# lmwdhr/ViT-CNN

Hardware: AMD Instinct MI355X
Metric: training patches/sec, 9×9 HSI(144)+LiDAR patch, batch 64, 1/2/4/8 GPU (higher is better)
Workload: dtype fp32; 1 GPU; ViT-CNN (Multimodality_Mamba) train step, Houston2013 shape 144+1 bands, 9x9, 16 classes; global_batch=64, per_gpu_batch=64, parallelism=dp1, launch=hipGraph (whole step)

## Files before the change

include/vitcnn.h:

```cpp
#ifndef VITCNN_H
#define VITCNN_H

#include <stddef.h>
#include <hip/hip_runtime_api.h>

#ifdef __cplusplus
#define VC_API extern "C" __attribute__((visibility("default")))
#else
#define VC_API __attribute__((visibility("default")))
#endif

VC_API int vc_gemm(int transA, int transB, int M, int N, int K, float alpha,
                   const float* A, long lda, long strideA, const float* B, long ldb, long strideB,
                   float beta, float* C, long ldc, long strideC, int batch,
                   const float* bias, const float* addend, long add_ld, int add_mod, int flags,
                   float* bias_grad, float* ws, long ws_floats, hipStream_t stream);
VC_API int vc_gemm_ex(int transA, int transB, int M, int N, int K, float alpha, const float* A, long lda,
                      long strideA, const float* B, long ldb, long strideB, float beta, float* C, long ldc,
                      long strideC, int batch, const float* bias, const float* addend, long add_ld, int add_mod,
                      int flags, float* bias_grad, float* ws, long ws_floats, unsigned int* tile_counters,
                      int n_counters, hipStream_t stream);

VC_API int vc_gemm_tune(int bm, int bn, int nsplit, int pf, int combine);

// ... 122 lines not shown
                                    float* dA_log, float* dDskip, float* dgate_logits, float* scratch,
                                    long scratch_floats, hipStream_t stream);
VC_API int vc_mamba_dirconv_bwd(int B, int L, int D, int ndir, const int* order, const int* inv_order,
                                const float* xz, const float* conv_w, const float* conv_b, float* du, float* dxz,
                                float* dconv_w, float* dconv_b, float* ws, long ws_floats, hipStream_t stream);
VC_API int vc_mamba_scan_fwd_fused(int B, int L, int D, int R, int ndir, const float* xz, const int* order,
                                   const float* conv_w, const float* conv_b, const float* x_proj_w,
                                   const float* dt_w, const float* dt_b, const float* A_log, const float* Dskip,
                                   float* u, float* xdbl, float* yp, float* ckpt, hipStream_t stream);
VC_API int vc_mamba_scan_bwd_fused(int B, int L, int D, int R, int ndir, const float* u, const float* xdbl,
                                   const int* order, const float* xz, const float* conv_w, const float* conv_b,
                                   const float* x_proj_w, const float* dt_w, const float* dt_b, const float* A_log,
                                   const float* Dskip, const float* gate_logits, const float* yp, const float* dyp,
                                   const float* ckpt, float* dpre, float* ddt_lin, float* dxdbl, float* conv_part,
                                   float* dA_log, float* dDskip, float* dgate_logits, float* ws, long ws_floats,
                                   hipStream_t stream);
VC_API int vc_mamba_dirconv_bwd_gather(int B, int L, int D, int ndir, const int* inv_order, const float* conv_w,
                                       const float* dpre, float* dxz, hipStream_t stream);
VC_API int vc_mamba_conv_params(int B, int D, int ndir, const float* conv_part, float* dconv_w, float* dconv_b,
                                hipStream_t stream);
VC_API int vc_mamba_bwd_params(int B, int D, int ndir, const float* gate_logits, const float* ws, const float* conv_part,
                               float* dA_log, float* dDskip, float* dgate_logits, float* dconv_w, float* dconv_b,
                               hipStream_t stream);

VC_API int vc_rowchain_front(int rows, int K0, int E, int N2, const float* x, const float* w_embed, const float* pos,
                             int L, float* t, const float* ln_w, const float* ln_b, float eps, float* xn, float* mean,
                             float* rstd, const float* w_proj, float* out, hipStream_t stream);
VC_API int vc_rowchain_back(int B, int L, int D, int ndir, const int* inv_order, const float* gate_logits,
                            const float* yp, const float* xz, float* ypsum, float* ysum, int E, const float* w_out,
                            const float* residual, float* t2, const float* ln_w, const float* ln_b, float eps,
                            float* g, float* mean, float* rstd, int N2, const float* w_proj, const float* b_proj,
                            float* out, hipStream_t stream);

VC_API int vc_rowchain_back_bwd(int rows, int Cout, int E, int D, const float* dcd, const float* w_cd, const float* t2,
                                const float* mean, const float* rstd, const float* ln_w, float* dt, float* ln_part,
                                const float* w_out, const float* xz, const float* ypsum, float* dyp, float* dxz,
                                hipStream_t stream);
VC_API int vc_rowchain_front_bwd(int rows, int K0, int E, int Cin, const float* dxz, const float* w_in, const float* t,
                                 const float* mean, const float* rstd, const float* ln_w, const float* res, float* dtt,
                                 float* ln_part, const float* w_embed, float* dx, float beta, const float* dx_add,
                                 hipStream_t stream);
VC_API int vc_rowchain_ln_params(int rows, int E, const float* ln_part, float* dw, float* db, float beta,
                                 hipStream_t stream);
VC_API int vc_rowchain_ln_part_floats(int rows, int E);

VC_API int vc_tl_ws_floats(int B, int HW, int S);
// ... 95 lines not shown
```

vit-cnn_amd/csrc/mamba.hip:

```cpp
#include "common.h"

namespace {

constexpr int NST = 16;

constexpr int DC_T = 8;
__global__ void dirconv_fwd_run(int total, FastDiv fD, FastDiv fC, FastDiv fB, int L, const int* __restrict__ order,
                                const float* __restrict__ xz, const float* __restrict__ cw,
                                const float* __restrict__ cb, float* __restrict__ u) {
  const int idx = blockIdx.x * blockDim.x + threadIdx.x;
  if (idx >= total) return;
  const int D = fD.div;
  int d, c, b;
  const int sc = fdivmod(idx, fD, d);
  const int sq = fdivmod(sc, fC, c);
  const int k = fdivmod(sq, fB, b);
  const int* ord = order + k * L;
  const float* xb = xz + (long)b * L * (2 * D) + d;
  const float w0 = cw[d * 4], w1 = cw[d * 4 + 1], w2 = cw[d * 4 + 2], w3 = cw[d * 4 + 3], bias = cb[d];
  const int t0 = c * DC_T;
  float x[DC_T + 3];
#pragma unroll
  for (int i = 0; i < DC_T + 3; ++i) {
    const int tau = t0 - 3 + i;
// ... 375 lines not shown
  const int l = threadIdx.x & 15;
  const bool b1 = l & 2;
  float z[2];
#if VC_DPP_PAIRWISE
  float y4[4];
#pragma unroll
  for (int j = 0; j < 4; ++j) y4[j] = dpp_pair_add<0>(v[j], v[j + 4]);
#pragma unroll
  for (int j = 0; j < 2; ++j) z[j] = dpp_pair_add<1>(y4[j], y4[j + 2]);
#else
  dpp_stage12(v, z[0], z[1]);
#endif
  const float keep = b1 ? z[1] : z[0], send = b1 ? z[0] : z[1];
  const float w = keep + dpp_mov<0x4E>(send);
  return w + dpp_mov<0xB1>(w);
}

struct FusedBwd {
  const float* xz;
  const float* conv_w;
  const float* conv_b;
  const float* wx;
  float* conv_part;
  int tail;
};

struct ScanBwdOut {
  float* du;
  float* ddtl;
  float* dxdbl;
  float* da_part;
  float* dd_part;
  float* dg_part;
};

template <int RT>
__device__ __forceinline__ void fused_bwd_tail(const ScanArgs& a, const FusedBwd& fb, const ScanBwdOut& o, int s,
                                               int b, const SeqLds& m, const int* ord, float* red, int Lp,
                                               int Dp) {
  const int R = RT ? RT : a.R, XW = R + 2 * NST, D = a.D, L = a.L;
  const int lane = threadIdx.x & 63, wave = threadIdx.x >> 6, nw = blockDim.x >> 6;
  const int r = lane & 15, g = lane >> 4;
  const int ntm = (Lp + 15) / 16, nkc = Dp / 16;
  const long base = (long)s * L;
  float* DX16 = red;
  float* wdt_lds = red + Lp * 16;
  {
    constexpr int WS = 8;
    float wv[WS];
#pragma unroll
    for (int j = 0; j < WS; ++j) {
      const int i = threadIdx.x + j * blockDim.x;
      wv[j] = i < D * R ? a.wdt[i] : 0.f;
    }
#pragma unroll
    for (int j = 0; j < WS; ++j) {
      const int i = threadIdx.x + j * blockDim.x;
      if (i < D * R) wdt_lds[i] = wv[j];
    }
  }
  __syncthreads();
  f32x4 avs[2][FMAX_KC];
  const int nu = (fb.tail & 2) ? 2 : 0;
#pragma unroll
  for (int u = 0; u < 2; ++u) {
    const int ta = 16 * (wave + u * nw) + r;
    const bool tok = ta < L;
// ... 9 lines not shown
  for (int u = 0; u < nu; ++u) {
    const int tm = wave + u * nw;
    if (tm >= ntm) break;
    const f32x4* av = avs[u];
    const bool jok = r < R;
    f32x4 acc = {0.f, 0.f, 0.f, 0.f};
#pragma unroll
    for (int kc = 0; kc < FMAX_KC; ++kc)
      if (kc < nkc) {
        const int k0 = 16 * kc + 4 * g;
        float bv[4];
#pragma unroll
        for (int e = 0; e < 4; ++e) bv[e] = (jok && k0 + e < D) ? wdt_lds[(k0 + e) * R + r] : 0.f;
        acc = __builtin_amdgcn_mfma_f32_16x16x4f32(av[kc].x, bv[0], acc, 0, 0, 0);
        acc = __builtin_amdgcn_mfma_f32_16x16x4f32(av[kc].y, bv[1], acc, 0, 0, 0);
        acc = __builtin_amdgcn_mfma_f32_16x16x4f32(av[kc].z, bv[2], acc, 0, 0, 0);
        acc = __builtin_amdgcn_mfma_f32_16x16x4f32(av[kc].w, bv[3], acc, 0, 0, 0);
      }
#pragma unroll
    for (int i = 0; i < 4; ++i) {
      const int t = 16 * tm + 4 * g + i;
      if (t < Lp) {
        DX16[t * 16 + r] = jok ? acc[i] : 0.f;
        if (jok && t < L) o.dxdbl[(base + t) * XW + r] = acc[i];
      }
    }
  }
  const int dl = 16 * wave + r;
  const bool dok = dl < D;
  const int dcl = dok ? dl : 0;
  f32x4 bw[3];
#pragma unroll
  for (int kc = 0; kc < 3; ++kc)
#pragma unroll
    for (int e = 0; e < 4; ++e) {
      const int jj = 4 * g + e;
      const int j = kc == 0 ? jj : R + 16 * (kc - 1) + jj;
      bw[kc][e] = (dok && (kc > 0 || jj < R)) ? fb.wx[(long)j * D + dcl] : 0.f;
    }
  __syncthreads();
  const unsigned lb = dok ? (unsigned)dl * 4u : 0x80000000u;
  const auto r_dp = buf_rsrc(o.du + base * D, (unsigned)(L * D * 4));
  const float w0 = cf_ld(fb.conv_w, dcl * 4, dok), w1 = cf_ld(fb.conv_w, dcl * 4 + 1, dok),
              w2 = cf_ld(fb.conv_w, dcl * 4 + 2, dok), w3 = cf_ld(fb.conv_w, dcl * 4 + 3, dok),
              bias = cf_ld(fb.conv_b, dcl, dok);
  const float* xb = fb.xz + (long)b * L * (2 * D) + dcl;
  float cacc[5] = {0.f, 0.f, 0.f, 0.f, 0.f};
// ... 40 lines not shown
          pre = fmaf(w2, xv[u][i + 2], pre);
          pre = fmaf(w3, xv[u][i + 3], pre);
          const float sg = sigmoid_f(pre);
          const float du = m.dts[(tq + i) * Dp + dl] + acc[i];
          const float gd = dok ? du * sg * (1.f + pre * (1.f - sg)) : 0.f;
          buf_st(r_dp, (unsigned)((tq + i) * D * 4) + lb, gd);
          cacc[4] += gd;
          cacc[0] += gd * xv[u][i];
          cacc[1] += gd * xv[u][i + 1];
          cacc[2] += gd * xv[u][i + 2];
          cacc[3] += gd * xv[u][i + 3];
        }
      }
    }
  }
#pragma unroll
  for (int e = 0; e < 5; ++e) cacc[e] = cross_row_sum(cacc[e]);
  if (g == 0 && dok) {
    float* cp = fb.conv_part + (long)s * 5 * D;
#pragma unroll
    for (int e = 0; e < 4; ++e) cp[dl * 4 + e] = cacc[e];
    cp[4 * D + dl] = cacc[4];
  }
}

template <int RT, bool BM, bool FUSE>
__global__ __launch_bounds__(512, 4) void scan_bwd(ScanArgs a, int ndir, const float* __restrict__ gate_logits,
                                                const float* __restrict__ yp, const float* __restrict__ dyp,
                                                const float* __restrict__ ckpt, ScanBwdOut o, int rbs,
                                                FusedBwd fb) {
  extern __shared__ __attribute__((aligned(16))) float smem[];
  const int R = RT ? RT : a.R;
  const int XW = R + 2 * NST;
  const int nseg = seg_count(a.L), Lp = nseg * SCK;
  const int nw = blockDim.x >> 6, Dp = nw * 16;
  const SeqLds m(smem, Lp, R, Dp);
  float* red = m.xr + Lp * R;
  const int nbuf = 2 * rbs;
  const int red_n = FUSE ? max(nbuf * nw * SCK * 32, Lp * 16 + a.D * R) : nbuf * nw * SCK * 32;
  int* ord = reinterpret_cast<int*>(red + red_n + nw);
  const int s = blockIdx.x, k = s / a.B, b = s - k * a.B;
  for (int t = threadIdx.x; t < a.L; t += blockDim.x) ord[t] = a.order[k * a.L + t];
  const int lane = threadIdx.x & 63, wave = threadIdx.x >> 6, q = lane >> 4, cl = lane & 15;
  const int d = wave * 16 + cl;
  const bool valid = d < a.D;
  const int dc = valid ? d : 0;
  const float g = gate_softmax(gate_logits, ndir, k);
  float A2[NQ];
#pragma unroll
  for (int j = 0; j < NQ; ++j) A2[j] = valid ? -__expf(a.alog[dc * NST + NQ * q + j]) * LOG2E : 0.f;
  const float Dd = valid ? a.dskip[dc] : 0.f;
  const long base = (long)s * a.L;
  const int vi = cl >> 1;
  const int col = vi < 4 ? NQ * q + vi : NST + NQ * q + vi - 4;
  const f2 A2v[2] = {f2{A2[0], A2[1]}, f2{A2[2], A2[3]}};
  f2 dh[2] = {f2{0.f, 0.f}, f2{0.f, 0.f}}, dAacc[2] = {f2{0.f, 0.f}, f2{0.f, 0.f}};
  float dD_acc = 0.f, dg_acc = 0.f;
  float hn[NQ], un[SCK], dn[SCK], yn[SCK];
  const unsigned seq_bytes = (unsigned)(a.L * a.D * 4);
  const auto r_u = buf_rsrc(a.u + base * a.D, seq_bytes);
  const auto r_yp = buf_rsrc(yp + base * a.D, seq_bytes);
  const auto r_dyp = buf_rsrc(dyp + (long)b * a.L * a.D, seq_bytes);
  const auto r_du = buf_rsrc(o.du + base * a.D, seq_bytes);
  const auto r_ddtl = buf_rsrc(o.ddtl + base * a.D, seq_bytes);
  const auto r_ck = buf_rsrc(ckpt + (long)s * nseg * NST * a.D, (unsigned)(nseg * NST * a.D * 4));
  const auto r_dx = buf_rsrc(o.dxdbl + base * XW, (unsigned)(a.L * XW * 4));
  const unsigned lane_b = valid ? (unsigned)d * 4u : 0x80000000u;
  auto load_seg = [&](int c) {
    const int t0 = c * SCK;
#pragma unroll
    for (int j = 0; j < NQ; ++j) hn[j] = buf_ld(r_ck, (unsigned)((c * NST + NQ * q + j) * a.D * 4) + lane_b);
#pragma unroll
    for (int i = 0; i < SCK; ++i) {
      const int t = t0 + i;
      const unsigned row = (unsigned)(t * a.D * 4) + lane_b;
      un[i] = buf_ld(r_u, row);
      dn[i] = buf_ld(r_dyp, (unsigned)((t < a.L ? ord[t] : a.L) * a.D * 4) + lane_b);
      yn[i] = buf_ld(r_yp, row);
    }
  };
  __syncthreads();
  load_seg(nseg - 1);
  stage_seq<RT>(a, s, m, Lp, Dp);
  for (int c = nseg - 1; c >= 0; --c) {
    const int t0 = c * SCK;
    f2 hs[SCK + 1][2];
    float uc[SCK], dyr[SCK];
    hs[0][0] = f2{hn[0], hn[1]};
    hs[0][1] = f2{hn[2], hn[3]};
// ... 73 lines not shown
        for (int ww = 1; ww < 8; ++ww)
          if (ww < nw) sum += pv[ww];
        buf_st(r_dx, (unsigned)(t * XW + R + cc) * 4u, sum);
        if (FUSE && t < Lp) (cc < NST ? m.Bs + t * NST + cc : m.Cs + t * NST + (cc - NST))[0] = sum;
      }
    }
  }
  dD_acc = cross_row_sum(dD_acc);
  if (valid) {
    float* dap = o.da_part + ((long)s * a.D + d) * NST + NQ * q;
#pragma unroll
    for (int j = 0; j < NQ; ++j) dap[j] = dAacc[j >> 1][j & 1] * A2[j] * LN2;
    if (q == 0) o.dd_part[(long)s * a.D + d] = dD_acc;
  }
  const float v = wave_sum(q == 0 ? dg_acc : 0.f);
  float* rg = red + red_n;
  if (lane == 0) rg[wave] = v;
  __syncthreads();
  if (threadIdx.x == 0) {
    float sum = 0.f;
    for (int ww = 0; ww < nw; ++ww) sum += rg[ww];
    o.dg_part[s] = sum;
  }
  if (FUSE && (fb.tail & 1)) fused_bwd_tail<RT>(a, fb, o, s, b, m, ord, red, Lp, Dp);
}

__global__ void gate_bwd(int total, FastDiv fD, const float* __restrict__ xz, const float* __restrict__ ypsum,
                         const float* __restrict__ dysum, float* __restrict__ dyp, float* __restrict__ dxz) {
  const int idx = blockIdx.x * blockDim.x + threadIdx.x;
  if (idx >= total) return;
  const int D = fD.div;
  int d;
  const int r = fdivmod(idx, fD, d);
  const float z = xz[(long)r * 2 * D + D + d];
  const float sg = sigmoid_f(z);
  const float g = dysum[idx];
  dyp[idx] = g * z * sg;
  dxz[(long)r * 2 * D + D + d] = g * ypsum[idx] * sg * (1.f + z * (1.f - sg));
}

template <int MAXK>
__global__ void combine_fwd(int total, FastDiv fD, FastDiv fL, int B, int ndir, const int* __restrict__ inv,
                            const float* __restrict__ logits, const float* __restrict__ y,
                            const float* __restrict__ xz, float* __restrict__ ypsum, float* __restrict__ out) {
  const int idx = blockIdx.x * blockDim.x + threadIdx.x;
  if (idx >= total) return;
  const int D = fD.div, L = fL.div;
// ... 37 lines not shown
      dg[kk] = s;
      gg[kk] = gate_softmax(logits, ndir, kk);
    }
  }
  __syncthreads();
  if (threadIdx.x < ndir) {
    float dot = 0.f;
    for (int i = 0; i < ndir; ++i) dot += gg[i] * dg[i];
    dlogits[threadIdx.x] = gg[threadIdx.x] * (dg[threadIdx.x] - dot);
  }
}

__global__ __launch_bounds__(256) void gate_grad(int ndir, int per_dir, const float* __restrict__ logits,
                                                 const float* __restrict__ part, float* __restrict__ dlogits) {
  __shared__ float dg[64], gg[64];
  gate_grad_body(ndir, per_dir, logits, part, dlogits, dg, gg);
}

__global__ __launch_bounds__(256) void mamba_params(int nseq, int D, int ndir, int ncb, const float* __restrict__ logits,
                                                    const float* __restrict__ pa, const float* __restrict__ pd,
                                                    const float* __restrict__ pg, const float* __restrict__ cp,
                                                    float* __restrict__ dA, float* __restrict__ dDs,
                                                    float* __restrict__ dgl, float* __restrict__ dcw,
                                                    float* __restrict__ dcb) {
  __shared__ float sh[16][17];
  __shared__ float dg[64], gg[64];
  if ((int)blockIdx.x == ncb) {
    gate_grad_body(ndir, nseq / ndir, logits, pg, dgl, dg, gg);
    return;
  }
  const int cl = threadIdx.x & 15, pl = threadIdx.x >> 4;
  const int c = blockIdx.x * 16 + cl;
  const float* src = nullptr;
  long stride = 0;
  float* dst = nullptr;
  int cc = 0;
  if (c < NST * D) src = pa, stride = (long)NST * D, dst = dA, cc = c;
  else if (c < (NST + 1) * D) src = pd, stride = D, dst = dDs, cc = c - NST * D;
  else if (c < (NST + 5) * D) src = cp, stride = 5L * D, dst = dcw, cc = c - (NST + 1) * D;
  else if (c < (NST + 6) * D) src = cp + 4L * D, stride = 5L * D, dst = dcb, cc = c - (NST + 5) * D;
  float s = 0.f;
  if (src) {
#pragma unroll 4
    for (int p = pl; p < nseq; p += 16) s += src[(long)p * stride + cc];
  }
  sh[pl][cl] = s;
  __syncthreads();
  if (pl == 0 && src) {
    float v = 0.f;
#pragma unroll
    for (int i = 0; i < 16; ++i) v += sh[i][cl];
    dst[cc] = v;
  }
}


template <int MAXK>
__global__ void dirconv_bwd_gather(int total, FastDiv fD, FastDiv fL, int B, int ndir, const int* __restrict__ inv,
                                   const float* __restrict__ cw, const float* __restrict__ dpre,
                                   float* __restrict__ dxz) {
  const int idx = blockIdx.x * blockDim.x + threadIdx.x;
  if (idx >= total) return;
  const int D = fD.div, L = fL.div;
// ... 160 lines not shown
                             const float* p_g, float* dA_log, float* dDskip, float* dgate_logits, float* scratch,
                             long scratch_floats, hipStream_t stream) {
  const int nseq = ndir * B;
  int rc = dA_log ? vc_colsum(nseq, D * NST, p_a, (long)D * NST, dA_log, 0.f, scratch, scratch_floats, stream) : 0;
  if (rc) return rc;
  rc = dDskip ? vc_colsum(nseq, D, p_d, (long)D, dDskip, 0.f, scratch, scratch_floats, stream) : 0;
  if (rc) return rc;
  if (!dgate_logits) return VC_OK;
  hipLaunchKernelGGL(gate_grad, dim3(1), dim3(256), 0, stream, ndir, B, gate_logits, p_g, dgate_logits);
  VC_CHECK_LAUNCH();
  return VC_OK;
}

static bool scan_fusable(int D, int R) { return D % 4 == 0 && R <= 16; }

static int scan_bwd_impl(int B, int L, int D, int R, int ndir, const float* u, const float* xdbl,
                         const int* order, const float* dt_w, const float* dt_b, const float* A_log,
                         const float* Dskip, const float* gate_logits, const float* y, const float* dyp,
                         const float* ckpt, float* du, float* ddt_lin, float* dxdbl, float* dA_log,
                         float* dDskip, float* dgate_logits, float* ws, long ws_floats, const FusedBwd* fb,
                         hipStream_t stream) {
  VC_REQUIRE(B > 0 && L > 0 && D > 0 && D <= 128 && R > 0 && R <= 64 && ndir > 0 && ndir <= 64);
  VC_REQUIRE(!fb || (ckpt && scan_fusable(D, R)));
  const int nseq = ndir * B;
  const long need_a = (long)nseq * D * NST, need_d = (long)nseq * D, need_g = nseq;
  long need_ck = 0;
  if (!ckpt) {
    const int n = vc_mamba_scan_ckpt_floats(B, L, D, ndir);
    VC_REQUIRE(n > 0);
    need_ck = n;
  }
  VC_REQUIRE(need_a + need_d + need_g + need_ck <= ws_floats);
  const int nw = vc_cdiv(D, 16);
  VC_REQUIRE(nw <= 8);
  int rbs = (int)std::max(1L, std::min(4L, vc_knob("VITCNN_SCAN_RBS", 2)));
  const long tail_n = fb ? (long)seg_count_h(L) * SCK * 16 + (long)D * R : 0;
  auto lds_bytes = [&](int r) {
    return sizeof(float) * (seq_lds_floats(L, R, nw * 16) + std::max<long>(2L * r * nw * SCK * 32, tail_n) + nw + L);
  };
  while (rbs > 1 && lds_bytes(rbs) > 160 * 1024 / 3 && lds_bytes(1) <= 160 * 1024 / 3) --rbs;
  const size_t sm = lds_bytes(rbs);
  VC_REQUIRE(sm <= 160 * 1024);
  VC_REQUIRE(!fb || (R <= 16 && (seg_count_h(L) * SCK + 15) / 16 <= 2 * nw));
  VC_REQUIRE_I32((long)nseq * L * (R + 2 * NST));
  float* p_a = ws;
  float* p_d = p_a + need_a;
  float* p_g = p_d + need_d;
  float* p_ck = p_g + need_g;
  float* p_rest = p_ck + need_ck;
  long rest = ws_floats - (need_a + need_d + need_g + need_ck);
  ScanArgs a{B, L, D, R, u, xdbl, order, dt_w, dt_b, A_log, Dskip};
  const dim3 grid(nseq), block(nw * 64);
  if (!ckpt) {
    const size_t smf = sizeof(float) * seq_lds_floats(L, R, nw * 16);
    if (R == 9) hipLaunchKernelGGL((scan_fwd<9, false>), grid, block, smf, stream, a, nullptr, p_ck, FusedFwd{});
    else if (R == 16) hipLaunchKernelGGL((scan_fwd<16, false>), grid, block, smf, stream, a, nullptr, p_ck, FusedFwd{});
    else hipLaunchKernelGGL((scan_fwd<0, false>), grid, block, smf, stream, a, nullptr, p_ck, FusedFwd{});
    VC_CHECK_LAUNCH();
    ckpt = p_ck;
  }
  ScanBwdOut o{du, ddt_lin, dxdbl, p_a, p_d, p_g};
  const bool bm = vc_knob("VITCNN_SCAN_SELECT_RS", 0) == 0;
#define VC_SCAN_BWD(RV)                                                                                     \
  do {                                                                                                      \
    if (fb) hipLaunchKernelGGL((scan_bwd<RV, true, true>), grid, block, sm, stream, a, ndir, gate_logits, y, dyp, ckpt, o, rbs, *fb); \
    else if (bm) hipLaunchKernelGGL((scan_bwd<RV, true, false>), grid, block, sm, stream, a, ndir, gate_logits, y, dyp, ckpt, o, rbs, FusedBwd{}); \
    else hipLaunchKernelGGL((scan_bwd<RV, false, false>), grid, block, sm, stream, a, ndir, gate_logits, y, dyp, ckpt, o, rbs, FusedBwd{}); \
  } while (0)
  if (R == 9) VC_SCAN_BWD(9);
  else if (R == 16) VC_SCAN_BWD(16);
  else VC_SCAN_BWD(0);
#undef VC_SCAN_BWD
  VC_CHECK_LAUNCH();
  return scan_param_reduce(B, D, ndir, gate_logits, p_a, p_d, p_g, dA_log, dDskip, dgate_logits, p_rest, rest, stream);
}

VC_API int vc_mamba_scan_bwd(int B, int L, int D, int R, int ndir, const float* u, const float* xdbl,
                             const int* order, const float* dt_w, const float* dt_b, const float* A_log,
                             const float* Dskip, const float* gate_logits, const float* y, const float* dyp,
                             const float* ckpt, float* du, float* ddt_lin, float* dxdbl, float* dA_log,
                             float* dDskip, float* dgate_logits, float* ws, long ws_floats, hipStream_t stream) {
  return scan_bwd_impl(B, L, D, R, ndir, u, xdbl, order, dt_w, dt_b, A_log, Dskip, gate_logits, y, dyp, ckpt, du,
                       ddt_lin, dxdbl, dA_log, dDskip, dgate_logits, ws, ws_floats, nullptr, stream);
}

VC_API int vc_mamba_scan_bwd_fused(int B, int L, int D, int R, int ndir, const float* u, const float* xdbl,
                                   const int* order, const float* xz, const float* conv_w, const float* conv_b,
                                   const float* x_proj_w, const float* dt_w, const float* dt_b, const float* A_log,
                                   const float* Dskip, const float* gate_logits, const float* y, const float* dyp,
                                   const float* ckpt, float* dpre, float* ddt_lin, float* dxdbl, float* conv_part,
                                   float* dA_log, float* dDskip, float* dgate_logits, float* ws, long ws_floats,
                                   hipStream_t stream) {
  VC_REQUIRE(xz && conv_w && conv_b && x_proj_w && conv_part);
  VC_REQUIRE_I32((long)B * L * 2 * D);
  const FusedBwd fb{xz, conv_w, conv_b, x_proj_w, conv_part, (int)vc_knob("VITCNN_SCAN_TAIL", 7)};
  return scan_bwd_impl(B, L, D, R, ndir, u, xdbl, order, dt_w, dt_b, A_log, Dskip, gate_logits, y, dyp, ckpt, dpre,
                       ddt_lin, dxdbl, dA_log, dDskip, dgate_logits, ws, ws_floats, &fb, stream);
}

VC_API int vc_mamba_scan_fwd_fused(int B, int L, int D, int R, int ndir, const float* xz, const int* order,
                                   const float* conv_w, const float* conv_b, const float* x_proj_w,
                                   const float* dt_w, const float* dt_b, const float* A_log, const float* Dskip,
                                   float* u, float* xdbl, float* y, float* ckpt, hipStream_t stream) {
  VC_REQUIRE(B > 0 && L > 0 && D > 0 && D <= 128 && R > 0 && R <= 64 && ndir > 0);
  VC_REQUIRE(xz && order && conv_w && conv_b && x_proj_w && u && xdbl && scan_fusable(D, R));
  const dim3 grid(ndir * B), block(vc_cdiv(D, 16) * 64);
  VC_REQUIRE(block.x <= 512);
  const size_t sm = sizeof(float) * (seq_lds_floats(L, R, block.x / 4) + L);
  VC_REQUIRE(sm <= 160 * 1024);
  VC_REQUIRE_I32((long)ndir * B * L * (R + 2 * NST));
  VC_REQUIRE_I32((long)B * L * 2 * D);
  const ScanArgs a{B, L, D, R, u, xdbl, order, dt_w, dt_b, A_log, Dskip};
  const FusedFwd f{xz, conv_w, conv_b, x_proj_w, u, xdbl};
  if (R == 9) hipLaunchKernelGGL((scan_fwd<9, true>), grid, block, sm, stream, a, y, ckpt, f);
  else if (R == 16) hipLaunchKernelGGL((scan_fwd<16, true>), grid, block, sm, stream, a, y, ckpt, f);
  else hipLaunchKernelGGL((scan_fwd<0, true>), grid, block, sm, stream, a, y, ckpt, f);
  VC_CHECK_LAUNCH();
  return VC_OK;
// ... 15 lines not shown
}

VC_API int vc_mamba_conv_params(int B, int D, int ndir, const float* conv_part, float* dconv_w, float* dconv_b,
                                hipStream_t stream) {
  VC_REQUIRE(B > 0 && D > 0 && ndir > 0 && conv_part && dconv_w && dconv_b);
  const int nseq = ndir * B;
  if (dconv_b == dconv_w + 4L * D) return launch_sum_rows(nseq, 5 * D, conv_part, 5L * D, 0L, dconv_w, 0.f, stream);
  const int rc = launch_sum_rows(nseq, 4 * D, conv_part, 5L * D, 0L, dconv_w, 0.f, stream);
  if (rc) return rc;
  return launch_sum_rows(nseq, D, conv_part, 5L * D, 4L * D, dconv_b, 0.f, stream);
}

VC_API int vc_mamba_bwd_params(int B, int D, int ndir, const float* gate_logits, const float* ws, const float* conv_part,
                               float* dA_log, float* dDskip, float* dgate_logits, float* dconv_w, float* dconv_b,
                               hipStream_t stream) {
  VC_REQUIRE(B > 0 && D > 0 && ndir > 0 && ndir <= 64 && gate_logits && ws && conv_part && dA_log && dDskip &&
             dgate_logits && dconv_w && dconv_b);
  const int nseq = ndir * B;
  const float* p_a = ws;
  const float* p_d = p_a + (long)nseq * D * NST;
  const float* p_g = p_d + (long)nseq * D;
  const int ncb = vc_cdiv((NST + 6) * D, 16);
  hipLaunchKernelGGL(mamba_params, dim3(ncb + 1), dim3(256), 0, stream, nseq, D, ndir, ncb, gate_logits, p_a, p_d,
                     p_g, conv_part, dA_log, dDskip, dgate_logits, dconv_w, dconv_b);
  VC_CHECK_LAUNCH();
  return VC_OK;
}

VC_API int vc_mamba_scan_bwd_params(int B, int D, int ndir, const float* gate_logits, const float* ws,
                                    float* dA_log, float* dDskip, float* dgate_logits, float* scratch,
                                    long scratch_floats, hipStream_t stream) {
  VC_REQUIRE(B > 0 && D > 0 && ndir > 0 && ws);
  const int nseq = ndir * B;
  const float* p_a = ws;
  const float* p_d = p_a + (long)nseq * D * NST;
  const float* p_g = p_d + (long)nseq * D;
  return scan_param_reduce(B, D, ndir, gate_logits, p_a, p_d, p_g, dA_log, dDskip, dgate_logits, scratch,
                           scratch_floats, stream);
}


VC_API int vc_mamba_dirconv_bwd(int B, int L, int D, int ndir, const int* order, const int* inv_order, const float* xz,
                                const float* conv_w, const float* conv_b, float* du, float* dxz,
                                float* dconv_w, float* dconv_b, float* ws, long ws_floats, hipStream_t stream) {
  VC_REQUIRE(B > 0 && L > 0 && D > 0 && ndir > 0);
  const long rows = (long)ndir * B * L;
  VC_REQUIRE_I32(rows * D);
// ... 24 lines not shown
```

vit-cnn_amd/vitcnn_amd/model.py:

```python
from __future__ import annotations

import contextlib
import ctypes
import math
import sys
import weakref
from typing import Dict

import torch
import torch.nn as nn

from ._lib import lib
from .flat import install_grad_views
from .layers import ConvBnReluParams, FusionParams, GlobalLocalParams
from .scan_orders import scan_orders

F32 = 4
LN_EPS = 1e-6
BN_EPS = 1e-5
BN_MOM = 0.1
NDIR = 10
N_SIDE = 3
_ONE_PARAM_REDUCE = True
WGRAD_LANE = 2
WGRAD1_LANE = 3
_IMPLICIT_CONV = False
_DEFER_WGRAD = True
_DEFER_WGRAD1 = False
SIDE_SCRATCH = 1 << 23
PARAM_ALIGN = 4
ALIGN_MIN = 64
GEMM_GROUP_BYTES = 16384
GEMM_MASK = 64
_GLOBAL_FIRST = False
_GEMM_BNSTATS = True
_PG_LANE2 = False
N_COUNTERS = 1 << 16

_SCAN_FUSED = True
_ROW_CHAIN = True
_GLF_FUSED = True
_TAP_DGRAD = False
_LANES = True
_LANES_BWD = True
_TRACER = None
_GROUP = True
# ... 1039 lines not shown
        YS, dYS = f(pfx + ".YS", rows * D), f(pfx + ".dYS", rows * D)
        U, XD, XZ = f(pfx + ".U", NDIR * rows * D), f(pfx + ".XD", NDIR * rows * XW), f(pfx + ".XZ", rows * 2 * D)
        Y, YP = f(pfx + ".Y", NDIR * rows * D), f(pfx + ".YP", rows * D)
        dU, dDTL = f(pfx + ".dU", NDIR * rows * D), f(pfx + ".dDTL", NDIR * rows * D)
        dXD, dXZ, dYP = f(pfx + ".dXD", NDIR * rows * XW), f(pfx + ".dXZ", rows * 2 * D), f(pfx + ".dYP", rows * D)
        if self._chain_back_bwd_ok(blk):
            part = f(pfx + ".ln1part", self.L.vc_rowchain_ln_part_floats(rows, E))
            self.L.vc_rowchain_back_bwd(rows, Cout, E, D, dCD, P[pfx + ".change_dim.weight"], T2, f(pfx + ".G.m", rows),
                                        f(pfx + ".G.r", rows), P[gv + ".ln1.weight"], dT, part,
                                        P[mx + ".out_proj.weight"], XZ, YP, dYP, dXZ, self.s)
            self.defer_wgrad(True, Cout, E, rows, dCD, Cout, Gm, E, G[pfx + ".change_dim.weight"], E,
                             G[pfx + ".change_dim.bias"])
            self._ln_params(gv + ".ln1", rows, E, part)
            self.defer_wgrad(True, E, D, rows, dT, E, YS, D, G[mx + ".out_proj.weight"], D)
        else:
            self.linear_bwd(pfx + ".change_dim.weight", pfx + ".change_dim.bias", dCD, rows, Cout, E, Gm, E, dG, 0.0,
                            defer=True)
            self.ln_bwd(gv + ".ln1", pfx + ".G", dG, T2, rows, E, dT, 0.0, defer=True)
            self.linear_bwd(mx + ".out_proj.weight", None, dT, rows, E, D, YS, D, dYS, 0.0, defer=True)
            self.L.vc_mamba_gate_bwd(B, L_, D, XZ, YP, dYS, dYP, dXZ, self.s)
        self.flush_wgrads()
        CKPb = f(pfx + ".CKP", self.L.vc_mamba_scan_ckpt_floats(B, L_, D, NDIR))
        if self.scan_fused:
            self._scan_bwd_fused(pfx, gv, mx, B, L_, D, R, XW, order, inv, CKPb)
            return self._block_bwd_tail(blk, pfx, gv, mx, B, L_, E, Cin, rows, X, dX, dT, e_ch)
        if self._deferring(True):
            nseq = NDIR * B
            spn = nseq * D * 16 + nseq * D + nseq
            sp = f(pfx + ".scanpart", spn)
            self.L.vc_mamba_scan_bwd(B, L_, D, R, NDIR, U, XD, order, P[mx + ".dt_proj.weight"],
                                     P[mx + ".dt_proj.bias"], P[mx + ".A_log"], P[mx + ".D"], P[gv + ".weights"], Y,
                                     dYP, CKPb, dU, dDTL, dXD, None, None, None, sp, spn, self.s)
            gl, ga, gd, gg = P[gv + ".weights"], G[mx + ".A_log"], G[mx + ".D"], G[gv + ".weights"]
            self.pending_wgrads.append(
                lambda: self.L.vc_mamba_scan_bwd_params(B, D, NDIR, gl, sp, ga, gd, gg, self.scr_p, self.scr_n,
                                                        self.s))
        else:
            self.L.vc_mamba_scan_bwd(B, L_, D, R, NDIR, U, XD, order, P[mx + ".dt_proj.weight"],
                                     P[mx + ".dt_proj.bias"], P[mx + ".A_log"], P[mx + ".D"], P[gv + ".weights"], Y,
                                     dYP, CKPb, dU, dDTL, dXD, G[mx + ".A_log"], G[mx + ".D"], G[gv + ".weights"],
                                     self.scr_p, self.scr_n, self.s)
        nr = NDIR * rows
        self.defer_wgrad(True, D, R, nr, dDTL, D, XD, XW, G[mx + ".dt_proj.weight"], R, G[mx + ".dt_proj.bias"])
        self.mm_nn(nr, R, D, dDTL, D, P[mx + ".dt_proj.weight"], R, dXD, XW)
        self.linear_bwd(mx + ".x_proj.weight", None, dXD, nr, XW, D, U, D, dU, 1.0, defer=True)
        self.L.vc_mamba_dirconv_bwd(B, L_, D, NDIR, order, inv, XZ, P[mx + ".conv1d.weight"], P[mx + ".conv1d.bias"],
                                    dU, dXZ, G[mx + ".conv1d.weight"], G[mx + ".conv1d.bias"], self.scr_p,
                                    self.scr_n, self.s)
        self._block_bwd_tail(blk, pfx, gv, mx, B, L_, E, Cin, rows, X, dX, dT, e_ch)

    def _scan_bwd_fused(self, pfx, gv, mx, B, L_, D, R, XW, order, inv, CKPb):
        P, G, f = self.P, self.G, self.ws.f
        rows = B * L_
        nr, nseq = NDIR * rows, NDIR * B
        U, XD, XZ = f(pfx + ".U", nr * D), f(pfx + ".XD", nr * XW), f(pfx + ".XZ", rows * 2 * D)
        Y, dYP = f(pfx + ".Y", nr * D), f(pfx + ".dYP", rows * D)
        dU, dDTL, dXD, dXZ = f(pfx + ".dU", nr * D), f(pfx + ".dDTL", nr * D), f(pfx + ".dXD", nr * XW), f(
            pfx + ".dXZ", rows * 2 * D)
        CP = f(pfx + ".convpart", nseq * 5 * D)
        defer = self._deferring(True)
        spn = nseq * D * 16 + nseq * D + nseq
        sp = f(pfx + ".scanpart", spn)
        gl, ga, gd, gg = P[gv + ".weights"], G[mx + ".A_log"], G[mx + ".D"], G[gv + ".weights"]
        self.L.vc_mamba_scan_bwd_fused(B, L_, D, R, NDIR, U, XD, order, XZ, P[mx + ".conv1d.weight"],
                                       P[mx + ".conv1d.bias"], P[mx + ".x_proj.weight"], P[mx + ".dt_proj.weight"],
                                       P[mx + ".dt_proj.bias"], P[mx + ".A_log"], P[mx + ".D"], gl, Y, dYP, CKPb, dU,
                                       dDTL, dXD, CP, None, None, None, sp, spn, self.s)
        cw, cb = G[mx + ".conv1d.weight"], G[mx + ".conv1d.bias"]
        if _ONE_PARAM_REDUCE:
            params = lambda: self.L.vc_mamba_bwd_params(B, D, NDIR, gl, sp, CP, ga, gd, gg, cw, cb, self.s)
        else:
            def params():
                self.L.vc_mamba_scan_bwd_params(B, D, NDIR, gl, sp, ga, gd, gg, self.scr_p, self.scr_n, self.s)
                self.L.vc_mamba_conv_params(B, D, NDIR, CP, cw, cb, self.s)
        if defer:
            self.pending_wgrads.append(params)
        else:
            params()
        self.L.vc_mamba_dirconv_bwd_gather(B, L_, D, NDIR, inv, P[mx + ".conv1d.weight"], dU, dXZ, self.s)
        self.defer_wgrad(True, D, R, nr, dDTL, D, XD, XW, G[mx + ".dt_proj.weight"], R, G[mx + ".dt_proj.bias"])
        self.defer_wgrad(True, XW, D, nr, dXD, XW, U, D, G[mx + ".x_proj.weight"], D)

    def _chain_ok(self, blk):
        E = blk.embed
        return (self.row_chain and blk.cin <= 256 and blk.cin % 4 == 0 and E <= 256 and E % 4 == 0
                and (E // 2) % 4 == 0 and blk.cout <= 256)

    def _chain_back_bwd_ok(self, blk):
        return self._chain_ok(blk) and blk.cout % 4 == 0

    def _ln_params(self, pfx, rows, E, part):
# ... 84 lines not shown
```

Before: 38990 patches/s.

## Fuse x_proj and dt_proj weight-gradient partials into the scan backward tail

Adds a WG variant of the fused scan backward kernel. Its tail uses MFMA to compute per-sequence partial weight gradients for x_proj (dt, B and C slices) and dt_proj, plus the dt bias sum, from data already resident in LDS. The extended params kernel then reduces these partials across sequences, so the separate deferred wgrad GEMMs and the dxdbl global write are dropped. This saves extra launches and traffic at the cost of more work and register pressure in the scan tail, plus a larger partial buffer.

```diff
diff --git a/include/vitcnn.h b/include/vitcnn.h
--- a/include/vitcnn.h
+++ b/include/vitcnn.h
@@ -168,6 +168,18 @@
 VC_API int vc_mamba_bwd_params(int B, int D, int ndir, const float* gate_logits, const float* ws, const float* conv_part,
                                float* dA_log, float* dDskip, float* dgate_logits, float* dconv_w, float* dconv_b,
                                hipStream_t stream);
+VC_API int vc_mamba_scan_wg_floats(int B, int D, int R, int ndir);
+VC_API int vc_mamba_scan_bwd_fused_wg(int B, int L, int D, int R, int ndir, const float* u, const float* xdbl,
+                                      const int* order, const float* xz, const float* conv_w, const float* conv_b,
+                                      const float* x_proj_w, const float* dt_w, const float* dt_b, const float* A_log,
+                                      const float* Dskip, const float* gate_logits, const float* yp, const float* dyp,
+                                      const float* ckpt, float* dpre, float* ddt_lin, float* dxdbl, float* conv_part,
+                                      float* wg_part, float* dA_log, float* dDskip, float* dgate_logits, float* ws,
+                                      long ws_floats, hipStream_t stream);
+VC_API int vc_mamba_bwd_params_wg(int B, int D, int R, int ndir, const float* gate_logits, const float* ws,
+                                  const float* conv_part, const float* wg_part, float* dA_log, float* dDskip,
+                                  float* dgate_logits, float* dconv_w, float* dconv_b, float* dx_proj_w, float* ddt_w,
+                                  float* ddt_b, hipStream_t stream);
 
 VC_API int vc_rowchain_front(int rows, int K0, int E, int N2, const float* x, const float* w_embed, const float* pos,
                              int L, float* t, const float* ln_w, const float* ln_b, float eps, float* xn, float* mean,
diff --git a/vit-cnn_amd/csrc/mamba.hip b/vit-cnn_amd/csrc/mamba.hip
--- a/vit-cnn_amd/csrc/mamba.hip
+++ b/vit-cnn_amd/csrc/mamba.hip
@@ -421,6 +421,7 @@
   const float* conv_b;
   const float* wx;
   float* conv_part;
+  float* wg_part;
   int tail;
 };
 
@@ -433,15 +434,21 @@
   float* dg_part;
 };
 
-template <int RT>
+static long wg_part_floats(int D, int R) { return (long)(R + 2 * NST) * D + (long)D * R + D; }
+
+template <int RT, bool WG>
 __device__ __forceinline__ void fused_bwd_tail(const ScanArgs& a, const FusedBwd& fb, const ScanBwdOut& o, int s,
                                                int b, const SeqLds& m, const int* ord, float* red, int Lp,
                                                int Dp) {
   const int R = RT ? RT : a.R, XW = R + 2 * NST, D = a.D, L = a.L;
-  const int lane = threadIdx.x & 63, wave = threadIdx.x >> 6, nw = blockDim.x >> 6;
+  int tid = threadIdx.x;
+  if (WG) asm volatile("" : "+v"(tid));
+  const int lane = tid & 63, wave = tid >> 6, nw = blockDim.x >> 6;
   const int r = lane & 15, g = lane >> 4;
   const int ntm = (Lp + 15) / 16, nkc = Dp / 16;
   const long base = (long)s * L;
+  const auto r_dx = buf_rsrc(WG && o.dxdbl ? o.dxdbl + base * XW : nullptr,
+                             WG && o.dxdbl ? (unsigned)(L * XW * 4) : 0u);
   float* DX16 = red;
   float* wdt_lds = red + Lp * 16;
   {
@@ -497,7 +504,10 @@
       const int t = 16 * tm + 4 * g + i;
       if (t < Lp) {
         DX16[t * 16 + r] = jok ? acc[i] : 0.f;
-        if (jok && t < L) o.dxdbl[(base + t) * XW + r] = acc[i];
+        if (jok && t < L) {
+          if (WG) buf_st(r_dx, (unsigned)(t * XW + r) * 4u, acc[i]);
+          else o.dxdbl[(base + t) * XW + r] = acc[i];
+        }
       }
     }
   }
@@ -584,9 +594,56 @@
     for (int e = 0; e < 4; ++e) cp[dl * 4 + e] = cacc[e];
     cp[4 * D + dl] = cacc[4];
   }
-}
-
-template <int RT, bool BM, bool FUSE>
+  if (!WG) return;
+  const bool jok = r < R;
+  const auto r_u = buf_rsrc(a.u + base * D, (unsigned)(L * D * 4));
+  const auto r_dd = buf_rsrc(o.ddtl + base * D, (unsigned)(L * D * 4));
+  const int rx = jok ? r : 0;
+  const int nks = Lp / 4;
+  f32x4 ax0 = {0.f, 0.f, 0.f, 0.f}, ax1 = ax0, ax2 = ax0, adt = ax0;
+  float bsum = 0.f;
+  constexpr int KS = 8;
+  for (int k0 = 0; k0 < nks; k0 += KS) {
+    float uv[KS], dv[KS];
+#pragma unroll
+    for (int e = 0; e < KS; ++e) {
+      const unsigned off = (unsigned)((4 * (k0 + e) + g) * D * 4) + lb;
+      uv[e] = buf_ld(r_u, off);
+      dv[e] = buf_ld(r_dd, off);
+    }
+#pragma unroll
+    for (int e = 0; e < KS; ++e) {
+      if (k0 + e >= nks) break;
+      const int t = 4 * (k0 + e) + g;
+      const bool tok = t < L;
+      const float a0 = tok ? DX16[t * 16 + r] : 0.f;
+      const float a1 = tok ? m.Bs[t * NST + r] : 0.f;
+      const float a2 = tok ? m.Cs[t * NST + r] : 0.f;
+      const float xv = tok && jok ? m.xr[t * R + rx] : 0.f;
+      ax0 = __builtin_amdgcn_mfma_f32_16x16x4f32(a0, uv[e], ax0, 0, 0, 0);
+      ax1 = __builtin_amdgcn_mfma_f32_16x16x4f32(a1, uv[e], ax1, 0, 0, 0);
+      ax2 = __builtin_amdgcn_mfma_f32_16x16x4f32(a2, uv[e], ax2, 0, 0, 0);
+      adt = __builtin_amdgcn_mfma_f32_16x16x4f32(dv[e], xv, adt, 0, 0, 0);
+      bsum += dv[e];
+    }
+  }
+  bsum = cross_row_sum(bsum);
+  float* wp = fb.wg_part + (long)s * ((long)XW * D + (long)D * R + D);
+#pragma unroll
+  for (int i = 0; i < 4; ++i) {
+    const int jj = 4 * g + i;
+    if (dok) {
+      if (jj < R) wp[jj * D + dl] = ax0[i];
+      wp[(R + jj) * D + dl] = ax1[i];
+      wp[(R + NST + jj) * D + dl] = ax2[i];
+    }
+    const int c = 16 * wave + jj;
+    if (c < D && jok) wp[XW * D + c * R + r] = adt[i];
+  }
+  if (g == 0 && dok) wp[XW * D + D * R + dl] = bsum;
+}
+
+template <int RT, bool BM, bool FUSE, bool WG = false>
 __global__ __launch_bounds__(512, 4) void scan_bwd(ScanArgs a, int ndir, const float* __restrict__ gate_logits,
                                                 const float* __restrict__ yp, const float* __restrict__ dyp,
                                                 const float* __restrict__ ckpt, ScanBwdOut o, int rbs,
@@ -626,7 +683,8 @@
   const auto r_du = buf_rsrc(o.du + base * a.D, seq_bytes);
   const auto r_ddtl = buf_rsrc(o.ddtl + base * a.D, seq_bytes);
   const auto r_ck = buf_rsrc(ckpt + (long)s * nseg * NST * a.D, (unsigned)(nseg * NST * a.D * 4));
-  const auto r_dx = buf_rsrc(o.dxdbl + base * XW, (unsigned)(a.L * XW * 4));
+  const bool has_dx = !WG || o.dxdbl;
+  const auto r_dx = buf_rsrc(has_dx ? o.dxdbl + base * XW : nullptr, has_dx ? (unsigned)(a.L * XW * 4) : 0u);
   const unsigned lane_b = valid ? (unsigned)d * 4u : 0x80000000u;
   auto load_seg = [&](int c) {
     const int t0 = c * SCK;
@@ -746,7 +804,7 @@
     for (int ww = 0; ww < nw; ++ww) sum += rg[ww];
     o.dg_part[s] = sum;
   }
-  if (FUSE && (fb.tail & 1)) fused_bwd_tail<RT>(a, fb, o, s, b, m, ord, red, Lp, Dp);
+  if (FUSE && (fb.tail & 1)) fused_bwd_tail<RT, WG>(a, fb, o, s, b, m, ord, red, Lp, Dp);
 }
 
 __global__ void gate_bwd(int total, FastDiv fD, const float* __restrict__ xz, const float* __restrict__ ypsum,
@@ -830,7 +888,9 @@
                                                     const float* __restrict__ pg, const float* __restrict__ cp,
                                                     float* __restrict__ dA, float* __restrict__ dDs,
                                                     float* __restrict__ dgl, float* __restrict__ dcw,
-                                                    float* __restrict__ dcb) {
+                                                    float* __restrict__ dcb, int R, const float* __restrict__ wg,
+                                                    float* __restrict__ dwx, float* __restrict__ dwdt,
+                                                    float* __restrict__ dbdt) {
   __shared__ float sh[16][17];
   __shared__ float dg[64], gg[64];
   if ((int)blockIdx.x == ncb) {
@@ -847,6 +907,13 @@
   else if (c < (NST + 1) * D) src = pd, stride = D, dst = dDs, cc = c - NST * D;
   else if (c < (NST + 5) * D) src = cp, stride = 5L * D, dst = dcw, cc = c - (NST + 1) * D;
   else if (c < (NST + 6) * D) src = cp + 4L * D, stride = 5L * D, dst = dcb, cc = c - (NST + 5) * D;
+  else if (wg) {
+    const int XW = R + 2 * NST, w = c - (NST + 6) * D;
+    stride = (long)XW * D + (long)D * R + D;
+    if (w < XW * D) src = wg, dst = dwx, cc = w;
+    else if (w < XW * D + D * R) src = wg + (long)XW * D, dst = dwdt, cc = w - XW * D;
+    else if (w < (int)stride) src = wg + (long)XW * D + (long)D * R, dst = dbdt, cc = w - XW * D - D * R;
+  }
   float s = 0.f;
   if (src) {
 #pragma unroll 4
@@ -1053,6 +1120,8 @@
                          hipStream_t stream) {
   VC_REQUIRE(B > 0 && L > 0 && D > 0 && D <= 128 && R > 0 && R <= 64 && ndir > 0 && ndir <= 64);
   VC_REQUIRE(!fb || (ckpt && scan_fusable(D, R)));
+  const bool wg = fb && fb->wg_part;
+  VC_REQUIRE(dxdbl || wg);
   const int nseq = ndir * B;
   const long need_a = (long)nseq * D * NST, need_d = (long)nseq * D, need_g = nseq;
   long need_ck = 0;
@@ -1094,7 +1163,8 @@
   const bool bm = vc_knob("VITCNN_SCAN_SELECT_RS", 0) == 0;
 #define VC_SCAN_BWD(RV)                                                                                     \
   do {                                                                                                      \
-    if (fb) hipLaunchKernelGGL((scan_bwd<RV, true, true>), grid, block, sm, stream, a, ndir, gate_logits, y, dyp, ckpt, o, rbs, *fb); \
+    if (wg) hipLaunchKernelGGL((scan_bwd<RV, true, true, true>), grid, block, sm, stream, a, ndir, gate_logits, y, dyp, ckpt, o, rbs, *fb); \
+    else if (fb) hipLaunchKernelGGL((scan_bwd<RV, true, true>), grid, block, sm, stream, a, ndir, gate_logits, y, dyp, ckpt, o, rbs, *fb); \
     else if (bm) hipLaunchKernelGGL((scan_bwd<RV, true, false>), grid, block, sm, stream, a, ndir, gate_logits, y, dyp, ckpt, o, rbs, FusedBwd{}); \
     else hipLaunchKernelGGL((scan_bwd<RV, false, false>), grid, block, sm, stream, a, ndir, gate_logits, y, dyp, ckpt, o, rbs, FusedBwd{}); \
   } while (0)
@@ -1124,7 +1194,28 @@
                                    hipStream_t stream) {
   VC_REQUIRE(xz && conv_w && conv_b && x_proj_w && conv_part);
   VC_REQUIRE_I32((long)B * L * 2 * D);
-  const FusedBwd fb{xz, conv_w, conv_b, x_proj_w, conv_part, (int)vc_knob("VITCNN_SCAN_TAIL", 7)};
+  const FusedBwd fb{xz, conv_w, conv_b, x_proj_w, conv_part, nullptr, (int)vc_knob("VITCNN_SCAN_TAIL", 7)};
+  return scan_bwd_impl(B, L, D, R, ndir, u, xdbl, order, dt_w, dt_b, A_log, Dskip, gate_logits, y, dyp, ckpt, dpre,
+                       ddt_lin, dxdbl, dA_log, dDskip, dgate_logits, ws, ws_floats, &fb, stream);
+}
+
+VC_API int vc_mamba_scan_wg_floats(int B, int D, int R, int ndir) {
+  if (B <= 0 || D <= 0 || R <= 0 || ndir <= 0) return -1;
+  const long n = (long)ndir * B * wg_part_floats(D, R);
+  return n < (1L << 31) ? (int)n : -1;
+}
+
+VC_API int vc_mamba_scan_bwd_fused_wg(int B, int L, int D, int R, int ndir, const float* u, const float* xdbl,
+                                      const int* order, const float* xz, const float* conv_w, const float* conv_b,
+                                      const float* x_proj_w, const float* dt_w, const float* dt_b, const float* A_log,
+                                      const float* Dskip, const float* gate_logits, const float* y, const float* dyp,
+                                      const float* ckpt, float* dpre, float* ddt_lin, float* dxdbl, float* conv_part,
+                                      float* wg_part, float* dA_log, float* dDskip, float* dgate_logits, float* ws,
+                                      long ws_floats, hipStream_t stream) {
+  VC_REQUIRE(xz && conv_w && conv_b && x_proj_w && conv_part && wg_part);
+  VC_REQUIRE_I32((long)B * L * 2 * D);
+  VC_REQUIRE(vc_mamba_scan_wg_floats(B, D, R, ndir) > 0);
+  const FusedBwd fb{xz, conv_w, conv_b, x_proj_w, conv_part, wg_part, 7};
   return scan_bwd_impl(B, L, D, R, ndir, u, xdbl, order, dt_w, dt_b, A_log, Dskip, gate_logits, y, dyp, ckpt, dpre,
                        ddt_lin, dxdbl, dA_log, dDskip, dgate_logits, ws, ws_floats, &fb, stream);
 }
@@ -1186,7 +1277,25 @@
   const float* p_g = p_d + (long)nseq * D;
   const int ncb = vc_cdiv((NST + 6) * D, 16);
   hipLaunchKernelGGL(mamba_params, dim3(ncb + 1), dim3(256), 0, stream, nseq, D, ndir, ncb, gate_logits, p_a, p_d,
-                     p_g, conv_part, dA_log, dDskip, dgate_logits, dconv_w, dconv_b);
+                     p_g, conv_part, dA_log, dDskip, dgate_logits, dconv_w, dconv_b, 0, nullptr, nullptr, nullptr, nullptr);
+  VC_CHECK_LAUNCH();
+  return VC_OK;
+}
+
+VC_API int vc_mamba_bwd_params_wg(int B, int D, int R, int ndir, const float* gate_logits, const float* ws,
+                                  const float* conv_part, const float* wg_part, float* dA_log, float* dDskip,
+                                  float* dgate_logits, float* dconv_w, float* dconv_b, float* dx_proj_w, float* ddt_w,
+                                  float* ddt_b, hipStream_t stream) {
+  VC_REQUIRE(B > 0 && D > 0 && R > 0 && ndir > 0 && ndir <= 64 && gate_logits && ws && conv_part && wg_part && dA_log &&
+             dDskip && dgate_logits && dconv_w && dconv_b && dx_proj_w && ddt_w && ddt_b);
+  VC_REQUIRE(vc_mamba_scan_wg_floats(B, D, R, ndir) > 0);
+  const int nseq = ndir * B;
+  const float* p_a = ws;
+  const float* p_d = p_a + (long)nseq * D * NST;
+  const float* p_g = p_d + (long)nseq * D;
+  const int ncb = vc_cdiv((long)(NST + 6) * D + wg_part_floats(D, R), 16);
+  hipLaunchKernelGGL(mamba_params, dim3(ncb + 1), dim3(256), 0, stream, nseq, D, ndir, ncb, gate_logits, p_a, p_d,
+                     p_g, conv_part, dA_log, dDskip, dgate_logits, dconv_w, dconv_b, R, wg_part, dx_proj_w, ddt_w, ddt_b);
   VC_CHECK_LAUNCH();
   return VC_OK;
 }
diff --git a/vit-cnn_amd/vitcnn_amd/model.py b/vit-cnn_amd/vitcnn_amd/model.py
--- a/vit-cnn_amd/vitcnn_amd/model.py
+++ b/vit-cnn_amd/vitcnn_amd/model.py
@@ -22,6 +22,7 @@
 NDIR = 10
 N_SIDE = 3
 _ONE_PARAM_REDUCE = True
+_SCAN_WGRAD_FUSED = 2
 WGRAD_LANE = 2
 WGRAD1_LANE = 3
 _IMPLICIT_CONV = False
@@ -1107,7 +1108,7 @@
         self.flush_wgrads()
         CKPb = f(pfx + ".CKP", self.L.vc_mamba_scan_ckpt_floats(B, L_, D, NDIR))
         if self.scan_fused:
-            self._scan_bwd_fused(pfx, gv, mx, B, L_, D, R, XW, order, inv, CKPb)
+            self._scan_bwd_fused(pfx, gv, mx, B, L_, D, R, XW, order, inv, CKPb, last=not dX)
             return self._block_bwd_tail(blk, pfx, gv, mx, B, L_, E, Cin, rows, X, dX, dT, e_ch)
         if self._deferring(True):
             nseq = NDIR * B
@@ -1134,24 +1135,40 @@
                                     self.scr_n, self.s)
         self._block_bwd_tail(blk, pfx, gv, mx, B, L_, E, Cin, rows, X, dX, dT, e_ch)
 
-    def _scan_bwd_fused(self, pfx, gv, mx, B, L_, D, R, XW, order, inv, CKPb):
+    def _scan_bwd_fused(self, pfx, gv, mx, B, L_, D, R, XW, order, inv, CKPb, last=False):
         P, G, f = self.P, self.G, self.ws.f
         rows = B * L_
         nr, nseq = NDIR * rows, NDIR * B
         U, XD, XZ = f(pfx + ".U", nr * D), f(pfx + ".XD", nr * XW), f(pfx + ".XZ", rows * 2 * D)
         Y, dYP = f(pfx + ".Y", nr * D), f(pfx + ".dYP", rows * D)
-        dU, dDTL, dXD, dXZ = f(pfx + ".dU", nr * D), f(pfx + ".dDTL", nr * D), f(pfx + ".dXD", nr * XW), f(
-            pfx + ".dXZ", rows * 2 * D)
+        dU, dDTL, dXZ = f(pfx + ".dU", nr * D), f(pfx + ".dDTL", nr * D), f(pfx + ".dXZ", rows * 2 * D)
         CP = f(pfx + ".convpart", nseq * 5 * D)
         defer = self._deferring(True)
         spn = nseq * D * 16 + nseq * D + nseq
         sp = f(pfx + ".scanpart", spn)
         gl, ga, gd, gg = P[gv + ".weights"], G[mx + ".A_log"], G[mx + ".D"], G[gv + ".weights"]
+        cw, cb = G[mx + ".conv1d.weight"], G[mx + ".conv1d.bias"]
+        if _SCAN_WGRAD_FUSED >= (1 if last else 2):
+            WG = f(pfx + ".wgpart", self.L.vc_mamba_scan_wg_floats(B, D, R, NDIR))
+            gwx, gwdt, gbdt = G[mx + ".x_proj.weight"], G[mx + ".dt_proj.weight"], G[mx + ".dt_proj.bias"]
+            self.L.vc_mamba_scan_bwd_fused_wg(B, L_, D, R, NDIR, U, XD, order, XZ, P[mx + ".conv1d.weight"],
+                                              P[mx + ".conv1d.bias"], P[mx + ".x_proj.weight"],
+                                              P[mx + ".dt_proj.weight"], P[mx + ".dt_proj.bias"], P[mx + ".A_log"],
+                                              P[mx + ".D"], gl, Y, dYP, CKPb, dU, dDTL, None, CP, WG, None, None, None,
+                                              sp, spn, self.s)
+            params = lambda: self.L.vc_mamba_bwd_params_wg(B, D, R, NDIR, gl, sp, CP, WG, ga, gd, gg, cw, cb, gwx,
+                                                           gwdt, gbdt, self.s)
+            if defer:
+                self.pending_wgrads.append(params)
+            else:
+                params()
+            self.L.vc_mamba_dirconv_bwd_gather(B, L_, D, NDIR, inv, P[mx + ".conv1d.weight"], dU, dXZ, self.s)
+            return
+        dXD = f(pfx + ".dXD", nr * XW)
         self.L.vc_mamba_scan_bwd_fused(B, L_, D, R, NDIR, U, XD, order, XZ, P[mx + ".conv1d.weight"],
                                        P[mx + ".conv1d.bias"], P[mx + ".x_proj.weight"], P[mx + ".dt_proj.weight"],
                                        P[mx + ".dt_proj.bias"], P[mx + ".A_log"], P[mx + ".D"], gl, Y, dYP, CKPb, dU,
                                        dDTL, dXD, CP, None, None, None, sp, spn, self.s)
-        cw, cb = G[mx + ".conv1d.weight"], G[mx + ".conv1d.bias"]
         if _ONE_PARAM_REDUCE:
             params = lambda: self.L.vc_mamba_bwd_params(B, D, NDIR, gl, sp, CP, ga, gd, gg, cw, cb, self.s)
         else:
```

Result: no change. 39250 patches/s (median of 6 runs) (+0.7%).
